# Aiqz/Edge-Enhancement

Measured on AMD Instinct MI355X. Metric: adversarial images/sec (PGD-10, resnet18_EE_square), higher is better.
Workload: dtype f32; 1 GPU; tiny_ee_at: resnet18_EE_square EE_BPDA3_AT_square, per-rank batch 100 x 3x64x64, PGD-10 eps 0.0627 alpha 0.0078, train step incl. SGD; global_batch=100, rccl_ranks=1, setup_steps=3, hip_graph=True, miopen_db=recorded, miopen_db_matched=True, full=False, probe_iters=0, device=AMD Radeon Graphics (gfx950:sramecc+:xnack-, 256 CUs)

## Files before the change

edge-enhancement_amd/csrc/ee_bn.hip:

```cpp
#include "ee_bn_math.hpp"

#include <type_traits>

namespace {

using namespace ee;

template <int NT>
__device__ __forceinline__ float block_sum(float v, float *scratch) {
#pragma unroll
    for (int off = 32; off > 0; off >>= 1) v += __shfl_xor(v, off);
    const int wave = threadIdx.x >> 6, lane = threadIdx.x & 63;
    __syncthreads();
    if (lane == 0) scratch[wave] = v;
    __syncthreads();
    float t = 0.0f;
#pragma unroll
    for (int w = 0; w < NT / 64; ++w) t += scratch[w];
    return t;
}

template <int NT, int NV>
__device__ __forceinline__ void block_sums(float (&v)[NV], float *scratch) {
#pragma unroll
// ... 644 lines not shown
    }
}

template <bool RELU>
__device__ __forceinline__ void slice_bwd_apply(const float *__restrict__ dy, const float *__restrict__ dy2, const float *__restrict__ y,
                                                const float *__restrict__ x, const float *__restrict__ gamma, const float *__restrict__ beta,
                                                float *__restrict__ dx, float *__restrict__ dres, BnShape s, int c, Slice sl, float mean, float invstd,
                                                float m1, float m2) {
    const float w = bn_gain(invstd, gamma, c);
    const float4 *dy4 = reinterpret_cast<const float4 *>(dy), *y4 = reinterpret_cast<const float4 *>(y), *x4 = reinterpret_cast<const float4 *>(x);
    float4 *dx4 = reinterpret_cast<float4 *>(dx), *dr4 = reinterpret_cast<float4 *>(dres);
    const bool want_x = dx != nullptr;
    const MaskArgs mk = mask_args(y, gamma, beta, invstd, c);
    for_slice(s, c, sl, [&](size_t o) { return bwd_load(dy4, reinterpret_cast<const float4 *>(dy2), y4, x4, o, RELU, want_x, mean, mk); }, [&](BwdIn in, size_t o) {
        const float4 g = masked_dz(in, RELU);
        if (dres) dr4[o] = g;
        if (dx) dx4[o] = bn_dx4(w, g, m1, bn_xhat4(in.x, mean, invstd), m2);
    });
}

template <bool RELU>
__global__ __launch_bounds__(SPLIT_NT) void bn_split_bwd_apply_kernel(const float *__restrict__ dy, const float *__restrict__ dy2, const float *__restrict__ y,
                                                                      const float *__restrict__ x, const float *__restrict__ beta, const float *__restrict__ gamma,
                                                                      const float *__restrict__ save_mean, const float *__restrict__ save_invstd,
                                                                      const float *__restrict__ running_mean,
                                                                      const float *__restrict__ running_var, float eps, int training,
                                                                      float *__restrict__ dx, float *__restrict__ dres, float *__restrict__ dgamma,
                                                                      float *__restrict__ dbeta, const float *__restrict__ ws, BnShape s, int S) {
    const int c = blockIdx.x, sl_i = blockIdx.y;
    const float n = static_cast<float>(s.B) * static_cast<float>(s.HW);
    const BnStats st = bn_known_stats(training, save_mean, save_invstd, running_mean, running_var, eps, c);
    __shared__ float parts[2 * SPLIT_MAX];
    float sdz, sdzx;
    sum_partials(ws, c, S, parts, sdz, sdzx);
    if (sl_i == 0 && threadIdx.x == 0) put_param_grads(dgamma, dbeta, c, sdz, sdzx);
    if (!dx && !dres) return;
    slice_bwd_apply<RELU>(dy, dy2, y, x, gamma, beta, dx, dres, s, c, my_slice(s.B * (s.HW / 4), S, sl_i), st.mean, st.invstd,
                          training ? sdz / n : 0.0f, training ? sdzx / n : 0.0f);
}

struct PoolShape {
    int B, C, H, W, OH, OW, IPW, G;
    int nosums;
};

struct Moments {
    float n, mean, m2;
};
__device__ __forceinline__ Moments merge(Moments a, Moments b) {
    if (b.n <= 0.0f) return a;
    if (a.n <= 0.0f) return b;
    const float n = a.n + b.n, d = b.mean - a.mean;
    return Moments{n, a.mean + d * (b.n / n), (a.m2 + b.m2) + d * d * (a.n * b.n / n)};
}
__global__ __launch_bounds__(SPLIT_NT) void bn_stats_finalize_kernel(const float *__restrict__ parts, int S, float eps, float momentum,
                                                                     float *running_mean, float *running_var, float *__restrict__ save_mean,
                                                                     float *__restrict__ save_invstd) {
    __shared__ Moments sh[SPLIT_NT / 64];
    const int c = blockIdx.x;
    const float *p = parts + static_cast<size_t>(c) * S * 3;
    Moments m{0.0f, 0.0f, 0.0f};
    for (int i = threadIdx.x; i < S; i += SPLIT_NT) {
        const float n = p[3 * i + 2];
        m = merge(m, Moments{n, n > 0.0f ? p[3 * i] / n : 0.0f, p[3 * i + 1]});
    }
#pragma unroll
    for (int off = 1; off < 64; off <<= 1) {
        Moments o{__shfl_xor(m.n, off), __shfl_xor(m.mean, off), __shfl_xor(m.m2, off)};
        m = (threadIdx.x & off) ? merge(o, m) : merge(m, o);
    }
    if ((threadIdx.x & 63) == 0) sh[threadIdx.x >> 6] = m;
    __syncthreads();
    if (threadIdx.x == 0) {
        Moments t = sh[0];
#pragma unroll
        for (int w = 1; w < SPLIT_NT / 64; ++w) t = merge(t, sh[w]);
        const float var = t.n > 0.0f ? t.m2 / t.n : 0.0f;
        bn_commit_stats(c, t.mean, var, bn_invstd(var, eps), t.n, momentum, save_mean, save_invstd, running_mean, running_var);
    }
}

constexpr int POOL_MERGE_MAX = 7;

__global__ __launch_bounds__(SPLIT_NT) void bn_pool_fwd_kernel(const float *__restrict__ x, const float *__restrict__ gamma,
                                                               const float *__restrict__ beta, float *running_mean, float *running_var,
                                                               float momentum, float eps, int training, float *__restrict__ yp,
                                                               uint8_t *__restrict__ code, float *__restrict__ save_mean,
                                                               float *__restrict__ save_invstd, const float *__restrict__ ws, PoolShape p, int S,
                                                               float *__restrict__ xa) {
    extern __shared__ __align__(16) float plane[];
    __shared__ float parts[2 * SPLIT_MAX];
    const int c = blockIdx.x, g = blockIdx.y;
    const int HW = p.H * p.W, HWq = HW / 4, OHW = p.OH * p.OW;
    const float n = static_cast<float>(p.B) * static_cast<float>(HW);
    float mean, invstd;
    if (training == 2) {
        mean = save_mean[c];
        invstd = save_invstd[c];
    } else if (training == 3) {
        const float *q = ws + static_cast<size_t>(c) * S * 3;
        float ps[POOL_MERGE_MAX], pm[POOL_MERGE_MAX], pn[POOL_MERGE_MAX];
#pragma unroll
        for (int j = 0; j < POOL_MERGE_MAX; ++j) {
            const int i = static_cast<int>(threadIdx.x) + j * SPLIT_NT, ic = i < S ? i : S - 1;
            ps[j] = q[3 * ic], pm[j] = q[3 * ic + 1], pn[j] = q[3 * ic + 2];
            if (i >= S) ps[j] = pm[j] = pn[j] = 0.0f;
        }
        float two[2] = {0.0f, 0.0f};
#pragma unroll
        for (int j = 0; j < POOL_MERGE_MAX; ++j) two[0] += ps[j], two[1] += pn[j];
        block_sums<SPLIT_NT, 2>(two, parts);
        const float cnt = two[1];
        mean = cnt > 0.0f ? two[0] / cnt : 0.0f;
        float m2 = 0.0f;
#pragma unroll
        for (int j = 0; j < POOL_MERGE_MAX; ++j) {
            const float d = (pn[j] > 0.0f ? ps[j] / pn[j] : mean) - mean;
            m2 += pm[j] + pn[j] * d * d;
        }
        __syncthreads();
        m2 = block_sum<SPLIT_NT>(m2, parts);
        const float var = cnt > 0.0f ? m2 / cnt : 0.0f;
        invstd = bn_invstd(var, eps);
        if (g == 0 && threadIdx.x == 0) bn_commit_stats(c, mean, var, invstd, cnt, momentum, save_mean, save_invstd, running_mean, running_var);
    } else if (training) {
        float var;
        combine_slices(ws, c, S, p.B * HWq, n, parts, mean, var);
        invstd = bn_invstd(var, eps);
        if (g == 0 && threadIdx.x == 0) bn_commit_stats(c, mean, var, invstd, n, momentum, save_mean, save_invstd, running_mean, running_var);
    } else {
        const BnStats st = bn_known_stats(0, save_mean, save_invstd, running_mean, running_var, eps, c);
        mean = st.mean, invstd = st.invstd;
    }
    const float a = bn_gain(invstd, gamma, c), b0 = bn_shift(beta, c);
    const int b_end = (g + 1) * p.IPW < p.B ? (g + 1) * p.IPW : p.B;
    for (int b = g * p.IPW; b < b_end; ++b) {
        const size_t pl = static_cast<size_t>(b) * p.C + c;
        const float4 *x4 = reinterpret_cast<const float4 *>(x) + pl * HWq;
        for (int q = threadIdx.x; q < HWq; q += SPLIT_NT) {
            reinterpret_cast<float4 *>(plane)[q] = relu_nan4(bn_affine4(x4[q], mean, a, b0));
        }
        __syncthreads();
        for (int o = threadIdx.x; o < OHW; o += SPLIT_NT) {
            const int oh = o / p.OW, ow = o - oh * p.OW;
            const int h0 = oh * 2 - 1, w0 = ow * 2 - 1;
            const int hs = h0 < 0 ? 0 : h0, wsx = w0 < 0 ? 0 : w0;
            const int he = h0 + 3 > p.H ? p.H : h0 + 3, we = w0 + 3 > p.W ? p.W : w0 + 3;
            float best = -INFINITY;
            int bc = (hs - h0) * 3 + (wsx - w0);
            for (int h = hs; h < he; ++h)
                for (int w = wsx; w < we; ++w) {
                    const float v = plane[h * p.W + w];
                    if (v > best || v != v) {
                        best = v;
                        bc = (h - h0) * 3 + (w - w0);
                    }
                }
            yp[pl * OHW + o] = best;
            code[pl * OHW + o] = static_cast<uint8_t>(bc);
            if (xa) xa[pl * OHW + o] = x[pl * HW + (h0 + bc / 3) * p.W + (w0 + bc % 3)];
        }
        __syncthreads();
    }
}

__global__ __launch_bounds__(SPLIT_NT) void bn_pool_bwd_sums_pooled_kernel(const float *__restrict__ dyp, const float *__restrict__ dyp2, const float *__restrict__ xa,
                                                                           const float *__restrict__ gamma, const float *__restrict__ beta,
                                                                           const float *__restrict__ save_mean, const float *__restrict__ save_invstd,
                                                                           float *__restrict__ ws, PoolShape p) {
    __shared__ float scratch[3 * (SPLIT_NT / 64)];
    const int c = blockIdx.x, g = blockIdx.y;
    const int OHW = p.OH * p.OW;
    const float mean = save_mean[c], invstd = save_invstd[c];
    const float a = bn_gain(invstd, gamma, c), b0 = bn_shift(beta, c);
    const int b_end = (g + 1) * p.IPW < p.B ? (g + 1) * p.IPW : p.B;
    float sdz = 0.0f, sdzx = 0.0f;
    for (int b = g * p.IPW; b < b_end; ++b) {
        const size_t pl = (static_cast<size_t>(b) * p.C + c) * OHW;
        for (int o0 = threadIdx.x; o0 < OHW; o0 += 4 * SPLIT_NT) {
            float gv[4], g2[4], xv[4];
#pragma unroll
            for (int u = 0; u < 4; ++u) {
                const int o = o0 + u * SPLIT_NT < OHW ? o0 + u * SPLIT_NT : OHW - 1;
                gv[u] = dyp[pl + o];
                g2[u] = dyp2 ? dyp2[pl + o] : 0.0f;
                xv[u] = xa[pl + o];
            }
#pragma unroll
            for (int u = 0; u < 4; ++u)
                if (o0 + u * SPLIT_NT < OHW) {
                    const float gg = dyp2 ? gv[u] + g2[u] : gv[u];
                    const float dz = mask1(gg, bn_affine(xv[u], mean, a, b0));
                    sdz += dz;
                    sdzx += dz * bn_xhat(xv[u], mean, invstd);
                }
        }
    }
    float two[2] = {sdz, sdzx};
    block_sums<SPLIT_NT, 2>(two, scratch);
    if (threadIdx.x == 0) {
        ws[(static_cast<size_t>(c) * p.G + g) * 2 + 0] = two[0];
        ws[(static_cast<size_t>(c) * p.G + g) * 2 + 1] = two[1];
    }
}

template <bool APPLY>
__global__ __launch_bounds__(SPLIT_NT) void bn_pool_bwd_kernel(const float *__restrict__ dyp, const float *__restrict__ dyp2, const uint8_t *__restrict__ code,
                                                               const float *__restrict__ x, const float *__restrict__ gamma,
                                                               const float *__restrict__ beta, const float *__restrict__ save_mean,
                                                               const float *__restrict__ save_invstd, const float *__restrict__ running_mean,
                                                               const float *__restrict__ running_var, float eps, int training,
                                                               float *__restrict__ dx, float *__restrict__ dgamma, float *__restrict__ dbeta,
                                                               float *__restrict__ ws, PoolShape p) {
    extern __shared__ __align__(16) float lds[];
    __shared__ float scratch[3 * (SPLIT_NT / 64)];
    const int c = blockIdx.x, g = blockIdx.y;
    const int HW = p.H * p.W, HWq = HW / 4, OHW = p.OH * p.OW, Wq = p.W / 4;
    float *gp = lds;
    uint8_t *cd = reinterpret_cast<uint8_t *>(lds + OHW);
    const BnStats st = bn_known_stats(training, save_mean, save_invstd, running_mean, running_var, eps, c);
    const float mean = st.mean, invstd = st.invstd;
    const float a = bn_gain(invstd, gamma, c), b0 = bn_shift(beta, c);
    float m1 = 0.0f, m2 = 0.0f;
    if (APPLY && !p.nosums) {
        __shared__ float parts[2 * SPLIT_MAX];
        float sdz, sdzx;
        sum_partials(ws, c, p.G, parts, sdz, sdzx);
        if (g == 0 && threadIdx.x == 0) put_param_grads(dgamma, dbeta, c, sdz, sdzx);
        if (!dx) return;
        const float n = static_cast<float>(p.B) * static_cast<float>(HW);
        m1 = training ? sdz / n : 0.0f;
        m2 = training ? sdzx / n : 0.0f;
    }
    float sdz = 0.0f, sdzx = 0.0f;
    const int b_end = (g + 1) * p.IPW < p.B ? (g + 1) * p.IPW : p.B;
    for (int b = g * p.IPW; b < b_end; ++b) {
        const size_t pl = static_cast<size_t>(b) * p.C + c;
        for (int o = threadIdx.x; o < OHW; o += SPLIT_NT) {
            gp[o] = dyp2 ? dyp[pl * OHW + o] + dyp2[pl * OHW + o] : dyp[pl * OHW + o];
            cd[o] = code[pl * OHW + o];
        }
        __syncthreads();
        const float4 *x4 = reinterpret_cast<const float4 *>(x) + pl * HWq;
        for (int q = threadIdx.x; q < HWq; q += SPLIT_NT) {
            const float4 v4 = x4[q];
            const int h = q / Wq, w_base = 4 * (q - h * Wq);
            const int oh0 = h >> 1, ow0 = w_base >> 1;
            const bool row2 = (h & 1) && oh0 + 1 < p.OH;
            float gv[2][3];
            int cv[2][3];
#pragma unroll
            for (int r = 0; r < 2; ++r)
#pragma unroll
                for (int k = 0; k < 3; ++k) {
                    const bool ok = (r == 0 || row2) && ow0 + k < p.OW;
                    const int idx = ok ? (oh0 + r) * p.OW + ow0 + k : 0;
                    gv[r][k] = ok ? gp[idx] : 0.0f;
                    cv[r][k] = ok ? cd[idx] : 255;
                }
            const float xv[4] = {v4.x, v4.y, v4.z, v4.w};
            float out[4];
#pragma unroll
            for (int v = 0; v < 4; ++v) {
                const int w = w_base + v, k0 = v >> 1;
                float acc = 0.0f;
#pragma unroll
                for (int r = 0; r < 2; ++r)
#pragma unroll
                    for (int kb = 0; kb < 2; ++kb) {
                        if (kb == 1 && !(v & 1)) continue;
                        const int k = k0 + kb;
                        const int want = (h - ((oh0 + r) * 2 - 1)) * 3 + (w - ((ow0 + k) * 2 - 1));
                        if (cv[r][k] == want) acc += gv[r][k];
                    }
                const float dz = mask1(acc, bn_affine(xv[v], mean, a, b0));
                const float xhat = bn_xhat(xv[v], mean, invstd);
                if (!APPLY) {
                    sdz += dz;
                    sdzx += dz * xhat;
                } else {
                    out[v] = bn_dx(a, dz, m1, xhat, m2);
                }
            }
            if (APPLY) reinterpret_cast<float4 *>(dx)[pl * HWq + q] = make_float4(out[0], out[1], out[2], out[3]);
        }
        __syncthreads();
    }
    if (!APPLY) {
        block_sum_pair<SPLIT_NT>(sdz, sdzx, scratch);
        if (threadIdx.x == 0) {
            ws[(static_cast<size_t>(c) * p.G + g) * 2 + 0] = sdz;
            ws[(static_cast<size_t>(c) * p.G + g) * 2 + 1] = sdzx;
        }
    }
}

inline bool pool_shape(int B, int C, int H, int W, PoolShape &p) {
    if (B < 1 || C < 1 || H < 1 || W < 4 || W % 4 || static_cast<int64_t>(H) * W > 16000) return false;
    if (static_cast<int64_t>(B) * C * H * W / 4 > 0x7fffffffLL) return false;
    const int ipw = (B + SPLIT_MAX - 1) / SPLIT_MAX;
    p = PoolShape{B, C, H, W, (H - 1) / 2 + 1, (W - 1) / 2 + 1, ipw, (B + ipw - 1) / ipw, 0};
    return true;
}

template <int NT, int VEC>
void launch_fwd(bool relu, hipStream_t st, const FwdArgs &a, BnShape s) {
    dispatch(relu, a.res != nullptr, [&](auto R, auto Q) {
        launch_fwd_args(bn_fwd_kernel<NT, VEC, decltype(R)::value, decltype(Q)::value>, dim3(static_cast<unsigned>(s.C)), dim3(NT), st, a, s);
    });
}

template <int NT, int VEC>
void launch_bwd(bool relu, hipStream_t st, const BwdArgs &a, BnShape s) {
    dispatch(relu, [&](auto R) { launch_bwd_args(bn_bwd_kernel<NT, VEC, decltype(R)::value>, dim3(static_cast<unsigned>(s.C)), dim3(NT), st, a, s); });
}


__global__ __launch_bounds__(64) void bn_moments_kernel(const float *__restrict__ ws, float *__restrict__ moments, BnShape s, int S) {
    const int c = blockIdx.x * 64 + threadIdx.x;
    if (c >= s.C) return;
    const float n = static_cast<float>(s.B) * static_cast<float>(s.HW);
    float mean, m2;
    combine_moments(ws + static_cast<size_t>(c) * S * 2, S, s.B * (s.HW / 4), n, mean, m2);
    moments[3 * c + 0] = mean;
    moments[3 * c + 1] = m2;
    moments[3 * c + 2] = n;
}

__global__ __launch_bounds__(64) void bn_sums_kernel(const float *__restrict__ ws, float *__restrict__ sums, int C, int S) {
    const int c = blockIdx.x * 64 + threadIdx.x;
    if (c >= C) return;
    float a = 0.0f, b = 0.0f;
    for (int i = 0; i < S; ++i) {
        a += ws[(static_cast<size_t>(c) * S + i) * 2];
        b += ws[(static_cast<size_t>(c) * S + i) * 2 + 1];
    }
    sums[2 * c] = a;
    sums[2 * c + 1] = b;
}

template <bool RELU, bool RES>
__global__ __launch_bounds__(SPLIT_NT) void bn_sync_apply_kernel(const float *__restrict__ x, const float *__restrict__ res, const float *__restrict__ gamma,
                                                                 const float *__restrict__ beta, const float *__restrict__ all_moments, int W,
                                                                 float *running_mean, float *running_var, float momentum, float eps,
                                                                 float *__restrict__ y, float *__restrict__ save_mean, float *__restrict__ save_invstd,
                                                                 BnShape s, int S) {
    const int c = blockIdx.x, sl_i = blockIdx.y;
    Moments t{0.0f, 0.0f, 0.0f};
    for (int r = 0; r < W; ++r) {
        const float *m = all_moments + (static_cast<size_t>(r) * s.C + c) * 3;
        t = merge(t, Moments{m[2], m[0], m[1]});
    }
    const float var = t.n > 0.0f ? t.m2 / t.n : 0.0f;
    const float mean = t.mean, invstd = bn_invstd(var, eps);
    if (sl_i == 0 && threadIdx.x == 0) bn_commit_stats(c, mean, var, invstd, t.n, momentum, save_mean, save_invstd, running_mean, running_var);
    slice_fwd_apply<RELU, RES>(x, res, y, s, c, my_slice(s.B * (s.HW / 4), S, sl_i), mean, bn_gain(invstd, gamma, c), bn_shift(beta, c));
}

template <bool RELU>
__global__ __launch_bounds__(SPLIT_NT) void bn_sync_bwd_apply_kernel(const float *__restrict__ dy, const float *__restrict__ dy2, const float *__restrict__ y,
                                                                     const float *__restrict__ x, const float *__restrict__ beta, const float *__restrict__ gamma,
                                                                     const float *__restrict__ save_mean, const float *__restrict__ save_invstd,
                                                                     const float *__restrict__ global_sums, float n_global, float *__restrict__ dx,
                                                                     float *__restrict__ dres, BnShape s, int S) {
    const int c = blockIdx.x, sl_i = blockIdx.y;
    slice_bwd_apply<RELU>(dy, dy2, y, x, gamma, beta, dx, dres, s, c, my_slice(s.B * (s.HW / 4), S, sl_i), save_mean[c], save_invstd[c],
                          global_sums[2 * c] / n_global, global_sums[2 * c + 1] / n_global);
}

inline bool al16(const void *q) { return !q || aligned16(q); }

inline bool stats_ptrs_ok(int training, const float *save_mean, const float *save_invstd, const float *running_mean, const float *running_var) {
    return training ? (save_mean && save_invstd) : (running_mean && running_var);
}

inline bool bn_args_settled(int B, int C, int HW, bool tensors, int training, const float *save_mean, const float *save_invstd, const float *running_mean,
                            const float *running_var, int &status) {
    status = EE_OK;
    if (B < 0 || C < 1 || HW < 1 || static_cast<int64_t>(B) * HW > 0x7fffffffLL) status = EE_ERR_SHAPE;
    else if (B == 0) return true;
    else if (!tensors || !stats_ptrs_ok(training, save_mean, save_invstd, running_mean, running_var)) status = EE_ERR_NULL;
    return status != EE_OK;
}

inline dim3 split_grid(int C, int S) { return dim3(static_cast<unsigned>(C), static_cast<unsigned>(S)); }
// ... 56 lines not shown
            EE_LAUNCH(bn_split_bwd_partial_kernel<decltype(R)::value>, split_grid(C, S), dim3(SPLIT_NT), 0, st, dy, dy2, y, x, gamma, beta, save_mean,
                      save_invstd, running_mean, running_var, eps, training, workspace, s, S);
            launch_bwd_args(bn_split_bwd_apply_kernel<decltype(R)::value>, split_grid(C, S), dim3(SPLIT_NT), st, a, static_cast<const float *>(workspace), s, S);
        });
    } else {
        dispatch(vec, big, [&](auto V, auto G) { launch_bwd<decltype(G)::value ? 1024 : 256, decltype(V)::value ? 4 : 1>(relu != 0, st, a, s); });
    }
    return launch_status();
}

EE_API int ee_bn_act_bwd_f32(const float *dy, const float *y, const float *x, const float *gamma, const float *save_mean,
                             const float *save_invstd, const float *running_mean, const float *running_var, float eps, int training, int relu,
                             float *dx, float *dresidual, float *dgamma, float *dbeta, float *workspace, int B, int C, int HW, void *stream) {
    if (relu && !y) return EE_ERR_NULL;
    return ee_bn_act_bwd2_f32(dy, nullptr, y, x, gamma, nullptr, save_mean, save_invstd, running_mean, running_var, eps, training, relu, dx, dresidual, dgamma,
                              dbeta, workspace, B, C, HW, stream);
}

EE_API int ee_bn_sum_act_fwd_f32(const float *x, const float *res, const float *gamma, const float *beta, float *running_mean, float *running_var,
                                 float momentum, float eps, int training, int relu, float *sum_out, float *y, float *save_mean, float *save_invstd,
                                 int B, int C, int HW, void *stream) {
    int status;
    if (bn_args_settled(B, C, HW, x && res && y, training, save_mean, save_invstd, running_mean, running_var, status)) return status;
    if (HW % 4 || !al16(x) || !al16(res) || !al16(y) || !al16(sum_out)) return EE_ERR_UNSUPPORTED;
    const BnShape s{B, C, HW};
    const FwdArgs a{x, res, gamma, beta, running_mean, running_var, momentum, eps, training, y, save_mean, save_invstd};
    hipStream_t st = as_stream(stream);
    if (!with_cached_cfg(cached_variant(static_cast<int64_t>(B) * (HW / 4), static_cast<int64_t>(B) * C * HW), [&](auto cfg) {
            launch_fwd_cached<decltype(cfg)::NT, decltype(cfg)::MAXV>(relu != 0, true, st, a, s, sum_out);
        }))
        return EE_ERR_UNSUPPORTED;
    return launch_status();
}

EE_API int ee_bn_sum_act_bwd_f32(const float *dy, const float *dy2, const float *y, const float *s, const float *gamma, const float *beta,
                                 const float *save_mean, const float *save_invstd, const float *running_mean, const float *running_var, float eps,
                                 int training, int relu, const float *ds_add, float *ds, float *dgamma, float *dbeta, int B, int C, int HW,
                                 void *stream) {
    int status;
    if (bn_args_settled(B, C, HW, dy && s && ds, training, save_mean, save_invstd, running_mean, running_var, status)) return status;
    if (HW % 4 || !al16(dy) || !al16(dy2) || !al16(y) || !al16(s) || !al16(ds_add) || !al16(ds)) return EE_ERR_UNSUPPORTED;
    const BnShape sh{B, C, HW};
    const BwdArgs a{dy, dy2, y, s, beta, gamma, save_mean, save_invstd, running_mean, running_var, eps, training, ds, nullptr, dgamma, dbeta};
    hipStream_t st = as_stream(stream);
    if (!with_cached_cfg(cached_variant(static_cast<int64_t>(B) * (HW / 4), static_cast<int64_t>(B) * C * HW), [&](auto cfg) {
            launch_bwd_cached<decltype(cfg)::NT, decltype(cfg)::MAXV>(relu != 0, st, a, sh, ds_add);
        }))
        return EE_ERR_UNSUPPORTED;
    return launch_status();
}

EE_API int ee_bn_relu_pool_workspace_floats(int B, int C, int H, int W) {
    PoolShape p;
    if (!pool_shape(B, C, H, W, p)) return 0;
    return C * SPLIT_MAX * 2;
}

static int bn_relu_pool_fwd_impl(const float *x, const float *gamma, const float *beta, float *running_mean, float *running_var,
                                 float momentum, float eps, int training, float *y_pool, uint8_t *code, float *x_argmax, float *save_mean,
                                 float *save_invstd, float *workspace, const float *conv_stats, int conv_stats_slices, int B, int C, int H,
                                 int W, void *stream) {
    if (B < 0 || C < 1 || H < 1 || W < 1) return EE_ERR_SHAPE;
    if (B == 0) return EE_OK;
    PoolShape p;
    if (!pool_shape(B, C, H, W, p)) return EE_ERR_UNSUPPORTED;
    if (!x || !y_pool || !code || !workspace) return EE_ERR_NULL;
    if (!stats_ptrs_ok(training, save_mean, save_invstd, running_mean, running_var)) return EE_ERR_NULL;
    if (!aligned16(x)) return EE_ERR_ALIGN;
    hipStream_t st = as_stream(stream);
    const BnShape s{B, C, H * W};
    const int S = split_slices(static_cast<int64_t>(B) * (H * W / 4));
    int mode = training ? 1 : 0;
    const float *wsk = workspace;
    int Sk = S;
    if (training && conv_stats && conv_stats_slices > 0 && conv_stats_slices <= POOL_MERGE_MAX * SPLIT_NT) {
        mode = 3, wsk = conv_stats, Sk = conv_stats_slices;
    } else if (training && conv_stats && conv_stats_slices > 0) {
        EE_LAUNCH(bn_stats_finalize_kernel, dim3(static_cast<unsigned>(C)), dim3(SPLIT_NT), 0, st, conv_stats, conv_stats_slices, eps, momentum, running_mean,
                  running_var, save_mean, save_invstd);
        mode = 2;
    } else if (training) {
        EE_LAUNCH(bn_split_stats_kernel, dim3(static_cast<unsigned>(C), static_cast<unsigned>(S)), dim3(SPLIT_NT), 0, st, x, workspace, s, S);
    }
    EE_LAUNCH(bn_pool_fwd_kernel, dim3(static_cast<unsigned>(C), static_cast<unsigned>(p.G)), dim3(SPLIT_NT), static_cast<size_t>(H) * W * sizeof(float), st,
              x, gamma, beta, running_mean, running_var, momentum, eps, mode, y_pool, code, save_mean, save_invstd, wsk, p, Sk, x_argmax);
    return launch_status();
}

EE_API int ee_bn_relu_pool_fwd_f32(const float *x, const float *gamma, const float *beta, float *running_mean, float *running_var,
                                   float momentum, float eps, int training, float *y_pool, uint8_t *code, float *save_mean,
                                   float *save_invstd, float *workspace, const float *conv_stats, int conv_stats_slices, int B, int C, int H,
                                   int W, void *stream) {
    return bn_relu_pool_fwd_impl(x, gamma, beta, running_mean, running_var, momentum, eps, training, y_pool, code, nullptr, save_mean, save_invstd, workspace,
                                 conv_stats, conv_stats_slices, B, C, H, W, stream);
}

EE_API int ee_bn_relu_pool_fwd_xa_f32(const float *x, const float *gamma, const float *beta, float *running_mean, float *running_var,
                                      float momentum, float eps, int training, float *y_pool, uint8_t *code, float *x_argmax, float *save_mean,
                                      float *save_invstd, float *workspace, const float *conv_stats, int conv_stats_slices, int B, int C, int H,
                                      int W, void *stream) {
    if (B > 0 && !x_argmax) return EE_ERR_NULL;
    return bn_relu_pool_fwd_impl(x, gamma, beta, running_mean, running_var, momentum, eps, training, y_pool, code, x_argmax, save_mean, save_invstd, workspace,
                                 conv_stats, conv_stats_slices, B, C, H, W, stream);
}

static int bn_relu_pool_bwd_impl(const float *dy_pool, const float *dy_pool2, const uint8_t *code, const float *x, const float *x_argmax, const float *gamma,
                                 const float *beta, const float *save_mean, const float *save_invstd, const float *running_mean, const float *running_var,
                                 float eps, int training, float *dx, float *dgamma, float *dbeta, float *workspace, int B, int C, int H,
                                 int W, void *stream) {
    if (B < 0 || C < 1 || H < 1 || W < 1) return EE_ERR_SHAPE;
    if (B == 0) return EE_OK;
    PoolShape p;
    if (!pool_shape(B, C, H, W, p)) return EE_ERR_UNSUPPORTED;
    if (!dy_pool || !code || !x || !workspace) return EE_ERR_NULL;
    if (!stats_ptrs_ok(training, save_mean, save_invstd, running_mean, running_var)) return EE_ERR_NULL;
    if (!aligned16(x) || (dx && !aligned16(dx))) return EE_ERR_ALIGN;
    hipStream_t st = as_stream(stream);
    const dim3 grid(static_cast<unsigned>(C), static_cast<unsigned>(p.G)), block(SPLIT_NT);
    const size_t lds = (static_cast<size_t>(p.OH) * p.OW * 5 + 15) / 16 * 16;
    p.nosums = (!training && !dgamma && !dbeta) ? 1 : 0;
    if (p.nosums && !dx) return EE_OK;
    if (!p.nosums && training && x_argmax)
        EE_LAUNCH(bn_pool_bwd_sums_pooled_kernel, grid, block, 0, st, dy_pool, dy_pool2, x_argmax, gamma, beta, save_mean, save_invstd, workspace, p);
    else if (!p.nosums)
        EE_LAUNCH((bn_pool_bwd_kernel<false>), grid, block, lds, st, dy_pool, dy_pool2, code, x, gamma, beta, save_mean, save_invstd, running_mean, running_var, eps,
                  training, dx, dgamma, dbeta, workspace, p);
    EE_LAUNCH((bn_pool_bwd_kernel<true>), grid, block, lds, st, dy_pool, dy_pool2, code, x, gamma, beta, save_mean, save_invstd, running_mean, running_var, eps,
              training, dx, dgamma, dbeta, workspace, p);
    return launch_status();
}

EE_API int ee_bn_relu_pool_bwd_f32(const float *dy_pool, const float *dy_pool2, const uint8_t *code, const float *x, const float *gamma, const float *beta,
                                   const float *save_mean, const float *save_invstd, const float *running_mean, const float *running_var,
                                   float eps, int training, float *dx, float *dgamma, float *dbeta, float *workspace, int B, int C, int H,
                                   int W, void *stream) {
    return bn_relu_pool_bwd_impl(dy_pool, dy_pool2, code, x, nullptr, gamma, beta, save_mean, save_invstd, running_mean, running_var, eps, training, dx, dgamma,
                                 dbeta, workspace, B, C, H, W, stream);
}

EE_API int ee_bn_relu_pool_bwd_xa_f32(const float *dy_pool, const float *dy_pool2, const uint8_t *code, const float *x, const float *x_argmax, const float *gamma,
                                      const float *beta, const float *save_mean, const float *save_invstd, const float *running_mean,
                                      const float *running_var, float eps, int training, float *dx, float *dgamma, float *dbeta, float *workspace, int B,
                                      int C, int H, int W, void *stream) {
    return bn_relu_pool_bwd_impl(dy_pool, dy_pool2, code, x, x_argmax, gamma, beta, save_mean, save_invstd, running_mean, running_var, eps, training, dx, dgamma,
                                 dbeta, workspace, B, C, H, W, stream);
}

EE_API int ee_bn_dual_supported(int B, int C, int HW) {
    if (B < 1 || C < 1 || HW < 1 || HW % 4) return 0;
    const int cv = cached_variant(static_cast<int64_t>(B) * (HW / 4), static_cast<int64_t>(B) * C * HW);
    return (cv == 1 || cv == 2) ? 1 : 0;
}

EE_API int ee_bn_dual_fwd_f32(const float *xa, const float *xb, const float *gamma_a, const float *beta_a, float *running_mean_a, float *running_var_a,
                              float momentum_a, float eps_a, float *save_mean_a, float *save_invstd_a, const float *gamma_b, const float *beta_b,
                              float *running_mean_b, float *running_var_b, float momentum_b, float eps_b, float *save_mean_b, float *save_invstd_b,
                              int training, float *y, int B, int C, int HW, void *stream) {
    if (B < 0 || C < 1 || HW < 1) return EE_ERR_SHAPE;
    if (B == 0) return EE_OK;
    if (!ee_bn_dual_supported(B, C, HW)) return EE_ERR_UNSUPPORTED;
    if (!xa || !xb || !y) return EE_ERR_NULL;
    if (training && (!save_mean_a || !save_invstd_a || !save_mean_b || !save_invstd_b)) return EE_ERR_NULL;
    if (!training && (!running_mean_a || !running_var_a || !running_mean_b || !running_var_b)) return EE_ERR_NULL;
    if (!aligned16(xa) || !aligned16(xb) || !aligned16(y)) return EE_ERR_ALIGN;
    const BnShape s{B, C, HW};
    const BnParams pa{gamma_a, beta_a, running_mean_a, running_var_a, momentum_a, eps_a, save_mean_a, save_invstd_a};
    const BnParams pb{gamma_b, beta_b, running_mean_b, running_var_b, momentum_b, eps_b, save_mean_b, save_invstd_b};
    const dim3 grid(static_cast<unsigned>(C)), block(256);
    if (cached_variant(static_cast<int64_t>(B) * (HW / 4), static_cast<int64_t>(B) * C * HW) == 1)
        EE_LAUNCH((bn_dual_fwd_cached_kernel<256, 2>), grid, block, 0, as_stream(stream), xa, xb, pa, pb, training, y, s);
    else
        EE_LAUNCH((bn_dual_fwd_cached_kernel<256, 7>), grid, block, 0, as_stream(stream), xa, xb, pa, pb, training, y, s);
    return launch_status();
}

EE_API int ee_bn_dual_bwd_f32(const float *dy, const float *dy2, const float *y, const float *xa, const float *xb, const float *gamma_a,
                              const float *save_mean_a, const float *save_invstd_a, const float *running_mean_a, const float *running_var_a,
                              float eps_a, const float *gamma_b, const float *save_mean_b, const float *save_invstd_b,
                              const float *running_mean_b, const float *running_var_b, float eps_b, int training, float *dxa, float *dxb,
                              float *dgamma_a, float *dbeta_a, float *dgamma_b, float *dbeta_b, int B, int C, int HW, void *stream) {
    if (B < 0 || C < 1 || HW < 1) return EE_ERR_SHAPE;
    if (B == 0) return EE_OK;
    if (!ee_bn_dual_supported(B, C, HW)) return EE_ERR_UNSUPPORTED;
    if (!dy || !y || !xa || !xb) return EE_ERR_NULL;
    if (training && (!save_mean_a || !save_invstd_a || !save_mean_b || !save_invstd_b)) return EE_ERR_NULL;
    if (!training && (!running_mean_a || !running_var_a || !running_mean_b || !running_var_b)) return EE_ERR_NULL;
    if (!aligned16(dy) || !al16(dy2) || !aligned16(y) || !aligned16(xa) || !aligned16(xb) || !al16(dxa) || !al16(dxb)) return EE_ERR_ALIGN;
    const BnShape s{B, C, HW};
    const BnParams pa{gamma_a, nullptr, const_cast<float *>(running_mean_a), const_cast<float *>(running_var_a), 0.0f, eps_a, const_cast<float *>(save_mean_a),
                      const_cast<float *>(save_invstd_a)};
    const BnParams pb{gamma_b, nullptr, const_cast<float *>(running_mean_b), const_cast<float *>(running_var_b), 0.0f, eps_b, const_cast<float *>(save_mean_b),
                      const_cast<float *>(save_invstd_b)};
    const dim3 grid(static_cast<unsigned>(C)), block(256);
    if (cached_variant(static_cast<int64_t>(B) * (HW / 4), static_cast<int64_t>(B) * C * HW) == 1)
        EE_LAUNCH((bn_dual_bwd_cached_kernel<256, 2>), grid, block, 0, as_stream(stream), dy, dy2, y, xa, xb, pa, pb, training, dxa, dxb, dgamma_a, dbeta_a,
                  dgamma_b, dbeta_b, s);
    else
        EE_LAUNCH((bn_dual_bwd_cached_kernel<256, 7>), grid, block, 0, as_stream(stream), dy, dy2, y, xa, xb, pa, pb, training, dxa, dxb, dgamma_a, dbeta_a,
                  dgamma_b, dbeta_b, s);
    return launch_status();
}

EE_API int ee_syncbn_workspace_floats(int B, int C, int HW) {
    if (B < 1 || C < 1 || HW < 1 || HW % 4) return 0;
    return C * split_slices(static_cast<int64_t>(B) * (HW / 4)) * 2;
}

static int syncbn_check(int B, int C, int HW) {
    if (B < 1 || C < 1 || HW < 1) return EE_ERR_SHAPE;
    if (HW % 4) return EE_ERR_UNSUPPORTED;
    if (static_cast<int64_t>(B) * C * HW / 4 > 0x7fffffffLL) return EE_ERR_SHAPE;
// ... 67 lines not shown
```

Measured before the change: 8809 adversarial images/s.

## Add double-buffered register-prefetch pipeline kernels for fused BN-ReLU-maxpool fwd/bwd

Adds pipelined variants of the fused BN+ReLU+maxpool forward and backward-apply kernels. Each block prefetches the next image's plane into registers while the current plane is pooled or back-propagated from a double-buffered LDS tile. The grid is also repartitioned to roughly five blocks per CU. This hides global load latency and evens out work across CUs, in exchange for more LDS and registers per block and more template instantiations. The new kernels are on by default and can be disabled with an environment variable.

Result: no change. 8875 adversarial images/s (median of 6 runs) (+0.7%).

```diff
diff --git a/edge-enhancement_amd/csrc/ee_bn.hip b/edge-enhancement_amd/csrc/ee_bn.hip
--- a/edge-enhancement_amd/csrc/ee_bn.hip
+++ b/edge-enhancement_amd/csrc/ee_bn.hip
@@ -750,18 +750,11 @@
 
 constexpr int POOL_MERGE_MAX = 7;
 
-__global__ __launch_bounds__(SPLIT_NT) void bn_pool_fwd_kernel(const float *__restrict__ x, const float *__restrict__ gamma,
-                                                               const float *__restrict__ beta, float *running_mean, float *running_var,
-                                                               float momentum, float eps, int training, float *__restrict__ yp,
-                                                               uint8_t *__restrict__ code, float *__restrict__ save_mean,
-                                                               float *__restrict__ save_invstd, const float *__restrict__ ws, PoolShape p, int S,
-                                                               float *__restrict__ xa) {
-    extern __shared__ __align__(16) float plane[];
-    __shared__ float parts[2 * SPLIT_MAX];
-    const int c = blockIdx.x, g = blockIdx.y;
-    const int HW = p.H * p.W, HWq = HW / 4, OHW = p.OH * p.OW;
+__device__ __forceinline__ void pool_fwd_stats(int training, int c, int g, const float *__restrict__ ws, int S, PoolShape p, float eps, float momentum,
+                                               float *running_mean, float *running_var, float *__restrict__ save_mean,
+                                               float *__restrict__ save_invstd, float *parts, float &mean, float &invstd) {
+    const int HW = p.H * p.W, HWq = HW / 4;
     const float n = static_cast<float>(p.B) * static_cast<float>(HW);
-    float mean, invstd;
     if (training == 2) {
         mean = save_mean[c];
         invstd = save_invstd[c];
@@ -800,6 +793,38 @@
         const BnStats st = bn_known_stats(0, save_mean, save_invstd, running_mean, running_var, eps, c);
         mean = st.mean, invstd = st.invstd;
     }
+}
+
+__device__ __forceinline__ int pool_fwd_window(const float *plane, PoolShape p, int o, float &best, int &bc) {
+    const int oh = o / p.OW, ow = o - oh * p.OW;
+    const int h0 = oh * 2 - 1, w0 = ow * 2 - 1;
+    const int hs = h0 < 0 ? 0 : h0, wsx = w0 < 0 ? 0 : w0;
+    const int he = h0 + 3 > p.H ? p.H : h0 + 3, we = w0 + 3 > p.W ? p.W : w0 + 3;
+    best = -INFINITY;
+    bc = (hs - h0) * 3 + (wsx - w0);
+    for (int h = hs; h < he; ++h)
+        for (int w = wsx; w < we; ++w) {
+            const float v = plane[h * p.W + w];
+            if (v > best || v != v) {
+                best = v;
+                bc = (h - h0) * 3 + (w - w0);
+            }
+        }
+    return (h0 + bc / 3) * p.W + (w0 + bc % 3);
+}
+
+__global__ __launch_bounds__(SPLIT_NT) void bn_pool_fwd_kernel(const float *__restrict__ x, const float *__restrict__ gamma,
+                                                               const float *__restrict__ beta, float *running_mean, float *running_var,
+                                                               float momentum, float eps, int training, float *__restrict__ yp,
+                                                               uint8_t *__restrict__ code, float *__restrict__ save_mean,
+                                                               float *__restrict__ save_invstd, const float *__restrict__ ws, PoolShape p, int S,
+                                                               float *__restrict__ xa) {
+    extern __shared__ __align__(16) float plane[];
+    __shared__ float parts[2 * SPLIT_MAX];
+    const int c = blockIdx.x, g = blockIdx.y;
+    const int HW = p.H * p.W, HWq = HW / 4, OHW = p.OH * p.OW;
+    float mean, invstd;
+    pool_fwd_stats(training, c, g, ws, S, p, eps, momentum, running_mean, running_var, save_mean, save_invstd, parts, mean, invstd);
     const float a = bn_gain(invstd, gamma, c), b0 = bn_shift(beta, c);
     const int b_end = (g + 1) * p.IPW < p.B ? (g + 1) * p.IPW : p.B;
     for (int b = g * p.IPW; b < b_end; ++b) {
@@ -810,25 +835,86 @@
         }
         __syncthreads();
         for (int o = threadIdx.x; o < OHW; o += SPLIT_NT) {
-            const int oh = o / p.OW, ow = o - oh * p.OW;
-            const int h0 = oh * 2 - 1, w0 = ow * 2 - 1;
-            const int hs = h0 < 0 ? 0 : h0, wsx = w0 < 0 ? 0 : w0;
-            const int he = h0 + 3 > p.H ? p.H : h0 + 3, we = w0 + 3 > p.W ? p.W : w0 + 3;
-            float best = -INFINITY;
-            int bc = (hs - h0) * 3 + (wsx - w0);
-            for (int h = hs; h < he; ++h)
-                for (int w = wsx; w < we; ++w) {
-                    const float v = plane[h * p.W + w];
-                    if (v > best || v != v) {
-                        best = v;
-                        bc = (h - h0) * 3 + (w - w0);
-                    }
-                }
+            float best;
+            int bc;
+            const int at = pool_fwd_window(plane, p, o, best, bc);
             yp[pl * OHW + o] = best;
             code[pl * OHW + o] = static_cast<uint8_t>(bc);
-            if (xa) xa[pl * OHW + o] = x[pl * HW + (h0 + bc / 3) * p.W + (w0 + bc % 3)];
+            if (xa) xa[pl * OHW + o] = x[pl * HW + at];
         }
         __syncthreads();
+    }
+}
+
+template <int R>
+__device__ __forceinline__ void pool_load_x(const float4 *__restrict__ x4, size_t pl, int HWq, float4 (&v)[R]) {
+#pragma unroll
+    for (int r = 0; r < R; ++r) {
+        const int q = static_cast<int>(threadIdx.x) + r * SPLIT_NT;
+        v[r] = x4[pl * HWq + (q < HWq ? q : HWq - 1)];
+    }
+}
+
+template <int R>
+__device__ __forceinline__ void pool_stage_y(float *y, float *raw, const float4 (&v)[R], int HWq, float mean, float a, float b0) {
+#pragma unroll
+    for (int r = 0; r < R; ++r) {
+        const int q = static_cast<int>(threadIdx.x) + r * SPLIT_NT;
+        if (q < HWq) {
+            reinterpret_cast<float4 *>(y)[q] = relu_nan4(bn_affine4(v[r], mean, a, b0));
+            if (raw) reinterpret_cast<float4 *>(raw)[q] = v[r];
+        }
+    }
+}
+
+template <int R>
+__global__ __launch_bounds__(SPLIT_NT) void bn_pool_fwd_pipe_kernel(const float *__restrict__ x, const float *__restrict__ gamma,
+                                                                    const float *__restrict__ beta, float *running_mean, float *running_var,
+                                                                    float momentum, float eps, int training, float *__restrict__ yp,
+                                                                    uint8_t *__restrict__ code, float *__restrict__ save_mean,
+                                                                    float *__restrict__ save_invstd, const float *__restrict__ ws, PoolShape p, int S,
+                                                                    float *__restrict__ xa) {
+    extern __shared__ __align__(16) float plane[];
+    __shared__ float parts[2 * SPLIT_MAX];
+    const int c = blockIdx.x, g = blockIdx.y;
+    const int HW = p.H * p.W, HWq = HW / 4, OHW = p.OH * p.OW;
+    const float4 *x4 = reinterpret_cast<const float4 *>(x);
+    const int b_begin = g * p.IPW, b_end = (g + 1) * p.IPW < p.B ? (g + 1) * p.IPW : p.B;
+    float4 v[R];
+    pool_load_x<R>(x4, static_cast<size_t>(b_begin) * p.C + c, HWq, v);
+    float mean, invstd;
+    pool_fwd_stats(training, c, g, ws, S, p, eps, momentum, running_mean, running_var, save_mean, save_invstd, parts, mean, invstd);
+    const float a = bn_gain(invstd, gamma, c), b0 = bn_shift(beta, c);
+    const int buf = xa ? 2 * HW : HW;
+    pool_stage_y<R>(plane, xa ? plane + HW : nullptr, v, HWq, mean, a, b0);
+    for (int b = b_begin, i = 0; b < b_end; ++b, i ^= 1) {
+        const float *y = plane + i * buf, *raw = y + HW;
+        float *yn = plane + (i ^ 1) * buf;
+        const int bn = b + 1 < b_end ? b + 1 : b;
+        pool_load_x<R>(x4, static_cast<size_t>(bn) * p.C + c, HWq, v);
+        __syncthreads();
+        float best[R], xav[R];
+        int bc[R];
+#pragma unroll
+        for (int r = 0; r < R; ++r) {
+            const int o = static_cast<int>(threadIdx.x) + r * SPLIT_NT;
+            best[r] = xav[r] = 0.0f, bc[r] = 0;
+            if (o < OHW) {
+                const int at = pool_fwd_window(y, p, o, best[r], bc[r]);
+                if (xa) xav[r] = raw[at];
+            }
+        }
+        if (b + 1 < b_end) pool_stage_y<R>(yn, xa ? yn + HW : nullptr, v, HWq, mean, a, b0);
+        const size_t pl = static_cast<size_t>(b) * p.C + c;
+#pragma unroll
+        for (int r = 0; r < R; ++r) {
+            const int o = static_cast<int>(threadIdx.x) + r * SPLIT_NT;
+            if (o < OHW) {
+                yp[pl * OHW + o] = best[r];
+                code[pl * OHW + o] = static_cast<uint8_t>(bc[r]);
+                if (xa) xa[pl * OHW + o] = xav[r];
+            }
+        }
     }
 }
 
@@ -872,6 +958,41 @@
     }
 }
 
+__device__ __forceinline__ void pool_bwd_quad(const float *gp, const uint8_t *cd, PoolShape p, int q, float4 v4, float mean, float a, float b0,
+                                              float (&dz)[4]) {
+    const int Wq = p.W / 4;
+    const int h = q / Wq, w_base = 4 * (q - h * Wq);
+    const int oh0 = h >> 1, ow0 = w_base >> 1;
+    const bool row2 = (h & 1) && oh0 + 1 < p.OH;
+    float gv[2][3];
+    int cv[2][3];
+#pragma unroll
+    for (int r = 0; r < 2; ++r)
+#pragma unroll
+        for (int k = 0; k < 3; ++k) {
+            const bool ok = (r == 0 || row2) && ow0 + k < p.OW;
+            const int idx = ok ? (oh0 + r) * p.OW + ow0 + k : 0;
+            gv[r][k] = ok ? gp[idx] : 0.0f;
+            cv[r][k] = ok ? cd[idx] : 255;
+        }
+    const float xv[4] = {v4.x, v4.y, v4.z, v4.w};
+#pragma unroll
+    for (int v = 0; v < 4; ++v) {
+        const int w = w_base + v, k0 = v >> 1;
+        float acc = 0.0f;
+#pragma unroll
+        for (int r = 0; r < 2; ++r)
+#pragma unroll
+            for (int kb = 0; kb < 2; ++kb) {
+                if (kb == 1 && !(v & 1)) continue;
+                const int k = k0 + kb;
+                const int want = (h - ((oh0 + r) * 2 - 1)) * 3 + (w - ((ow0 + k) * 2 - 1));
+                if (cv[r][k] == want) acc += gv[r][k];
+            }
+        dz[v] = mask1(acc, bn_affine(xv[v], mean, a, b0));
+    }
+}
+
 template <bool APPLY>
 __global__ __launch_bounds__(SPLIT_NT) void bn_pool_bwd_kernel(const float *__restrict__ dyp, const float *__restrict__ dyp2, const uint8_t *__restrict__ code,
                                                                const float *__restrict__ x, const float *__restrict__ gamma,
@@ -883,7 +1004,7 @@
     extern __shared__ __align__(16) float lds[];
     __shared__ float scratch[3 * (SPLIT_NT / 64)];
     const int c = blockIdx.x, g = blockIdx.y;
-    const int HW = p.H * p.W, HWq = HW / 4, OHW = p.OH * p.OW, Wq = p.W / 4;
+    const int HW = p.H * p.W, HWq = HW / 4, OHW = p.OH * p.OW;
     float *gp = lds;
     uint8_t *cd = reinterpret_cast<uint8_t *>(lds + OHW);
     const BnStats st = bn_known_stats(training, save_mean, save_invstd, running_mean, running_var, eps, c);
@@ -912,42 +1033,17 @@
         const float4 *x4 = reinterpret_cast<const float4 *>(x) + pl * HWq;
         for (int q = threadIdx.x; q < HWq; q += SPLIT_NT) {
             const float4 v4 = x4[q];
-            const int h = q / Wq, w_base = 4 * (q - h * Wq);
-            const int oh0 = h >> 1, ow0 = w_base >> 1;
-            const bool row2 = (h & 1) && oh0 + 1 < p.OH;
-            float gv[2][3];
-            int cv[2][3];
-#pragma unroll
-            for (int r = 0; r < 2; ++r)
-#pragma unroll
-                for (int k = 0; k < 3; ++k) {
-                    const bool ok = (r == 0 || row2) && ow0 + k < p.OW;
-                    const int idx = ok ? (oh0 + r) * p.OW + ow0 + k : 0;
-                    gv[r][k] = ok ? gp[idx] : 0.0f;
-                    cv[r][k] = ok ? cd[idx] : 255;
-                }
             const float xv[4] = {v4.x, v4.y, v4.z, v4.w};
-            float out[4];
+            float dz[4], out[4];
+            pool_bwd_quad(gp, cd, p, q, v4, mean, a, b0, dz);
 #pragma unroll
             for (int v = 0; v < 4; ++v) {
-                const int w = w_base + v, k0 = v >> 1;
-                float acc = 0.0f;
-#pragma unroll
-                for (int r = 0; r < 2; ++r)
-#pragma unroll
-                    for (int kb = 0; kb < 2; ++kb) {
-                        if (kb == 1 && !(v & 1)) continue;
-                        const int k = k0 + kb;
-                        const int want = (h - ((oh0 + r) * 2 - 1)) * 3 + (w - ((ow0 + k) * 2 - 1));
-                        if (cv[r][k] == want) acc += gv[r][k];
-                    }
-                const float dz = mask1(acc, bn_affine(xv[v], mean, a, b0));
                 const float xhat = bn_xhat(xv[v], mean, invstd);
                 if (!APPLY) {
-                    sdz += dz;
-                    sdzx += dz * xhat;
+                    sdz += dz[v];
+                    sdzx += dz[v] * xhat;
                 } else {
-                    out[v] = bn_dx(a, dz, m1, xhat, m2);
+                    out[v] = bn_dx(a, dz[v], m1, xhat, m2);
                 }
             }
             if (APPLY) reinterpret_cast<float4 *>(dx)[pl * HWq + q] = make_float4(out[0], out[1], out[2], out[3]);
@@ -959,6 +1055,99 @@
         if (threadIdx.x == 0) {
             ws[(static_cast<size_t>(c) * p.G + g) * 2 + 0] = sdz;
             ws[(static_cast<size_t>(c) * p.G + g) * 2 + 1] = sdzx;
+        }
+    }
+}
+
+template <int R>
+__device__ __forceinline__ void pool_load_bwd(const float *__restrict__ dyp, const float *__restrict__ dyp2, const uint8_t *__restrict__ code,
+                                              const float4 *__restrict__ x4, size_t pl, int OHW, int HWq, float (&g1)[R], float (&g2)[R],
+                                              uint8_t (&cr)[R], float4 (&xv)[R]) {
+#pragma unroll
+    for (int r = 0; r < R; ++r) {
+        const int o1 = static_cast<int>(threadIdx.x) + r * SPLIT_NT, o = o1 < OHW ? o1 : OHW - 1;
+        g1[r] = dyp[pl * OHW + o];
+        g2[r] = dyp2 ? dyp2[pl * OHW + o] : 0.0f;
+        cr[r] = code[pl * OHW + o];
+    }
+    pool_load_x<R>(x4, pl, HWq, xv);
+}
+
+template <int R>
+__device__ __forceinline__ void pool_stage_grad(float *gp, const float *dyp2, const float (&g1)[R], const float (&g2)[R], const uint8_t (&cr)[R], int OHW) {
+    uint8_t *cd = reinterpret_cast<uint8_t *>(gp + OHW);
+#pragma unroll
+    for (int r = 0; r < R; ++r) {
+        const int o = static_cast<int>(threadIdx.x) + r * SPLIT_NT;
+        if (o < OHW) {
+            gp[o] = dyp2 ? g1[r] + g2[r] : g1[r];
+            cd[o] = cr[r];
+        }
+    }
+}
+
+template <int R>
+__global__ __launch_bounds__(SPLIT_NT) void bn_pool_bwd_pipe_kernel(const float *__restrict__ dyp, const float *__restrict__ dyp2,
+                                                                    const uint8_t *__restrict__ code, const float *__restrict__ x,
+                                                                    const float *__restrict__ gamma, const float *__restrict__ beta,
+                                                                    const float *__restrict__ save_mean, const float *__restrict__ save_invstd,
+                                                                    const float *__restrict__ running_mean, const float *__restrict__ running_var,
+                                                                    float eps, int training, float *__restrict__ dx, float *__restrict__ dgamma,
+                                                                    float *__restrict__ dbeta, const float *__restrict__ ws, PoolShape p, int S) {
+    extern __shared__ __align__(16) float lds[];
+    const int c = blockIdx.x, g = blockIdx.y;
+    const int HW = p.H * p.W, HWq = HW / 4, OHW = p.OH * p.OW;
+    const int buf = (OHW * 5 + 15) / 16 * 4;
+    const float4 *x4 = reinterpret_cast<const float4 *>(x);
+    const int b_begin = g * p.IPW, b_end = (g + 1) * p.IPW < p.B ? (g + 1) * p.IPW : p.B;
+    float g1[R], g2[R];
+    uint8_t cr[R];
+    float4 xn[R], xc[R];
+    pool_load_bwd<R>(dyp, dyp2, code, x4, static_cast<size_t>(b_begin) * p.C + c, OHW, HWq, g1, g2, cr, xn);
+    const BnStats st = bn_known_stats(training, save_mean, save_invstd, running_mean, running_var, eps, c);
+    const float mean = st.mean, invstd = st.invstd;
+    const float a = bn_gain(invstd, gamma, c), b0 = bn_shift(beta, c);
+    float m1 = 0.0f, m2 = 0.0f;
+    if (!p.nosums) {
+        __shared__ float parts[2 * SPLIT_MAX];
+        float sdz, sdzx;
+        sum_partials(ws, c, S, parts, sdz, sdzx);
+        if (g == 0 && threadIdx.x == 0) put_param_grads(dgamma, dbeta, c, sdz, sdzx);
+        if (!dx) return;
+        const float n = static_cast<float>(p.B) * static_cast<float>(HW);
+        m1 = training ? sdz / n : 0.0f;
+        m2 = training ? sdzx / n : 0.0f;
+    }
+    pool_stage_grad<R>(lds, dyp2, g1, g2, cr, OHW);
+#pragma unroll
+    for (int r = 0; r < R; ++r) xc[r] = xn[r];
+    for (int b = b_begin, i = 0; b < b_end; ++b, i ^= 1) {
+        const float *gp = lds + i * buf;
+        const uint8_t *cd = reinterpret_cast<const uint8_t *>(gp + OHW);
+        const int bn = b + 1 < b_end ? b + 1 : b;
+        pool_load_bwd<R>(dyp, dyp2, code, x4, static_cast<size_t>(bn) * p.C + c, OHW, HWq, g1, g2, cr, xn);
+        __syncthreads();
+        float4 out[R];
+#pragma unroll
+        for (int r = 0; r < R; ++r) {
+            const int q = static_cast<int>(threadIdx.x) + r * SPLIT_NT;
+            out[r] = zero4();
+            if (q < HWq) {
+                const float xv[4] = {xc[r].x, xc[r].y, xc[r].z, xc[r].w};
+                float dz[4], o4[4];
+                pool_bwd_quad(gp, cd, p, q, xc[r], mean, a, b0, dz);
+#pragma unroll
+                for (int v = 0; v < 4; ++v) o4[v] = bn_dx(a, dz[v], m1, bn_xhat(xv[v], mean, invstd), m2);
+                out[r] = make_float4(o4[0], o4[1], o4[2], o4[3]);
+            }
+        }
+        if (b + 1 < b_end) pool_stage_grad<R>(lds + (i ^ 1) * buf, dyp2, g1, g2, cr, OHW);
+        const size_t pl = static_cast<size_t>(b) * p.C + c;
+#pragma unroll
+        for (int r = 0; r < R; ++r) {
+            const int q = static_cast<int>(threadIdx.x) + r * SPLIT_NT;
+            if (q < HWq) reinterpret_cast<float4 *>(dx)[pl * HWq + q] = out[r];
+            xc[r] = xn[r];
         }
     }
 }
@@ -969,6 +1158,35 @@
     const int ipw = (B + SPLIT_MAX - 1) / SPLIT_MAX;
     p = PoolShape{B, C, H, W, (H - 1) / 2 + 1, (W - 1) / 2 + 1, ipw, (B + ipw - 1) / ipw, 0};
     return true;
+}
+
+inline bool pool_pipe_on() {
+    const char *e = getenv("EEADV_POOL_PIPE");
+    return !(e && e[0] == '0');
+}
+
+inline int pool_pipe_regs(const PoolShape &p, size_t lds_bytes) {
+    const int HWq = p.H * p.W / 4, OHW = p.OH * p.OW, m = HWq > OHW ? HWq : OHW;
+    if (!pool_pipe_on() || lds_bytes + 1024 > 65536) return 0;
+    return m <= SPLIT_NT ? 1 : (m <= 2 * SPLIT_NT ? 2 : (m <= 4 * SPLIT_NT ? 4 : 0));
+}
+
+inline PoolShape pool_pipe_partition(PoolShape p) {
+    const int64_t grid = 5 * static_cast<int64_t>(device_cus());
+    const int64_t ipw = (static_cast<int64_t>(p.B) * p.C + grid - 1) / grid;
+    p.IPW = static_cast<int>(ipw > p.B ? p.B : ipw);
+    p.G = (p.B + p.IPW - 1) / p.IPW;
+    return p;
+}
+
+template <class F>
+bool with_pool_regs(int regs, F f) {
+    switch (regs) {
+        case 1: f(std::integral_constant<int, 1>{}); return true;
+        case 2: f(std::integral_constant<int, 2>{}); return true;
+        case 4: f(std::integral_constant<int, 4>{}); return true;
+        default: return false;
+    }
 }
 
 template <int NT, int VEC>
@@ -1191,8 +1409,14 @@
     } else if (training) {
         EE_LAUNCH(bn_split_stats_kernel, dim3(static_cast<unsigned>(C), static_cast<unsigned>(S)), dim3(SPLIT_NT), 0, st, x, workspace, s, S);
     }
-    EE_LAUNCH(bn_pool_fwd_kernel, dim3(static_cast<unsigned>(C), static_cast<unsigned>(p.G)), dim3(SPLIT_NT), static_cast<size_t>(H) * W * sizeof(float), st,
-              x, gamma, beta, running_mean, running_var, momentum, eps, mode, y_pool, code, save_mean, save_invstd, wsk, p, Sk, x_argmax);
+    const size_t plane_bytes = static_cast<size_t>(H) * W * sizeof(float), pipe_bytes = (x_argmax ? 4 : 2) * plane_bytes;
+    if (!with_pool_regs(pool_pipe_regs(p, pipe_bytes), [&](auto R) {
+            const PoolShape pp = pool_pipe_partition(p);
+            EE_LAUNCH(bn_pool_fwd_pipe_kernel<decltype(R)::value>, dim3(static_cast<unsigned>(C), static_cast<unsigned>(pp.G)), dim3(SPLIT_NT), pipe_bytes, st,
+                      x, gamma, beta, running_mean, running_var, momentum, eps, mode, y_pool, code, save_mean, save_invstd, wsk, pp, Sk, x_argmax);
+        }))
+        EE_LAUNCH(bn_pool_fwd_kernel, dim3(static_cast<unsigned>(C), static_cast<unsigned>(p.G)), dim3(SPLIT_NT), plane_bytes, st, x, gamma, beta,
+                  running_mean, running_var, momentum, eps, mode, y_pool, code, save_mean, save_invstd, wsk, p, Sk, x_argmax);
     return launch_status();
 }
 
@@ -1234,8 +1458,13 @@
     else if (!p.nosums)
         EE_LAUNCH((bn_pool_bwd_kernel<false>), grid, block, lds, st, dy_pool, dy_pool2, code, x, gamma, beta, save_mean, save_invstd, running_mean, running_var, eps,
                   training, dx, dgamma, dbeta, workspace, p);
-    EE_LAUNCH((bn_pool_bwd_kernel<true>), grid, block, lds, st, dy_pool, dy_pool2, code, x, gamma, beta, save_mean, save_invstd, running_mean, running_var, eps,
-              training, dx, dgamma, dbeta, workspace, p);
+    if (!with_pool_regs(pool_pipe_regs(p, 2 * lds), [&](auto R) {
+            const PoolShape pp = pool_pipe_partition(p);
+            EE_LAUNCH(bn_pool_bwd_pipe_kernel<decltype(R)::value>, dim3(static_cast<unsigned>(C), static_cast<unsigned>(pp.G)), block, 2 * lds, st, dy_pool,
+                      dy_pool2, code, x, gamma, beta, save_mean, save_invstd, running_mean, running_var, eps, training, dx, dgamma, dbeta, workspace, pp, p.G);
+        }))
+        EE_LAUNCH((bn_pool_bwd_kernel<true>), grid, block, lds, st, dy_pool, dy_pool2, code, x, gamma, beta, save_mean, save_invstd, running_mean, running_var,
+                  eps, training, dx, dgamma, dbeta, workspace, p);
     return launch_status();
 }
 
```
